# Gabrielcb/DaliID

Hardware: AMD Instinct MI355X
Metric: images/sec (train step) (higher is better)
Workload: dtype bf16; 1 GPU; configs[1]: ResNet-50 ReID bf16 256x128, PK batch 16x16=256 per GPU, center+proxy heads, Adam, EMA; global_batch=256, per_gpu_batch=256, parallelism=dp1

## Files before the change

daliid_amd/_lib.py:

```python
import ctypes
import os
import threading

import torch

_HERE = os.path.dirname(os.path.abspath(__file__))
LIB_PATH = os.environ.get("DALIID_LIB") or os.path.join(_HERE, "libdaliid_hip.so")

c_void_p, c_int, c_float, c_size_t = ctypes.c_void_p, ctypes.c_int, ctypes.c_float, ctypes.c_size_t


class DaliError(RuntimeError):
    pass


_SIGNATURES = {
    "dali_version": [],
    "dali_last_error": [],
    "dali_ctx_create": [c_int, ctypes.POINTER(c_void_p)],
    "dali_ctx_destroy": [c_void_p],
    "dali_ctx_reserve": [c_void_p, c_size_t],
    "dali_comm_unique_id": [c_void_p],
    "dali_ctx_comm_init": [c_void_p, c_void_p, c_int, c_int],
    "dali_ctx_comm_destroy": [c_void_p],
# ... 47 lines not shown
    "dali_linear_wgrad": [c_void_p] * 6 + [c_int] * 3,
    "dali_vit_patchify": [c_void_p, c_void_p, c_void_p] + [c_int] * 5 + [c_void_p],
    "dali_vit_assemble_tokens": [c_void_p] * 5 + [c_int] * 3 + [c_void_p],
    "dali_vit_assemble_tokens_bwd": [c_void_p] * 3 + [c_int] * 3 + [c_void_p] * 3,
    "dali_layernorm_fwd": [c_void_p] * 5 + [c_int, c_int, c_float] + [c_void_p] * 3,
    "dali_layernorm_bwd": [c_void_p] * 8 + [c_int, c_int] + [c_void_p] * 3,
    "dali_attention_fwd": [c_void_p] * 3 + [c_int] * 4 + [c_float, c_void_p, c_void_p],
    "dali_attention_bwd": [c_void_p] * 6 + [c_int] * 4 + [c_float, c_void_p],
    "dali_center_loss_fwd": [c_void_p] * 6 + [c_float, c_int, c_int, c_void_p, c_void_p],
    "dali_center_loss_bwd": [c_void_p] * 6 + [c_float, c_int, c_int, c_void_p, c_float, c_void_p],
    "dali_proxy_loss_fwd": [c_void_p] * 6 + [c_float, c_int, c_int] + [c_void_p] * 5,
    "dali_proxy_loss_bwd": [c_void_p] * 5 + [c_int, c_int, c_void_p, c_float, c_int, c_void_p],
    "dali_proxy_kmax": [],
    "dali_adam_step": [c_void_p] * 6 + [ctypes.c_int64, c_float, c_float, c_float, c_float, c_float, c_int, c_float, c_void_p],
    "dali_ema_update": [c_void_p, c_void_p, c_void_p, c_void_p, ctypes.c_int64, c_float],
    "dali_triplet_loss_fwd": [c_void_p, c_void_p, c_void_p, c_void_p, c_void_p, c_float, c_int, c_void_p, c_void_p, c_void_p, c_void_p,
                              c_void_p],
    "dali_triplet_loss_bwd": [c_void_p, c_void_p, c_void_p, c_void_p, c_int, c_void_p, c_float, c_void_p],
    "dali_pairdist_blend": [c_void_p, c_void_p, c_void_p, c_void_p, c_int, c_int, c_int, c_int, c_int, c_void_p, c_void_p, c_void_p,
                            c_void_p, c_void_p],
    "dali_class_targets": [c_void_p, c_void_p, c_void_p, c_int, c_int, c_void_p, c_void_p, c_int, c_void_p, c_int, c_void_p, c_void_p,
                           c_void_p, c_void_p],
    "dali_resize_bicubic_u8": [c_void_p] * 7 + [c_int, c_int, c_void_p, c_void_p, c_int, c_void_p, c_void_p, c_int, c_int, c_int, c_void_p],
    "dali_augment_batch": [c_void_p, c_void_p, c_void_p, c_void_p, c_int, c_int, c_int, ctypes.POINTER(c_float), ctypes.POINTER(c_float), c_void_p],
    "dali_gemm_profile_begin": [c_void_p, c_int],
    "dali_gemm_profile_end": [c_void_p, c_void_p, c_void_p, c_void_p],
    "dali_resnet_create": [c_void_p, c_void_p, ctypes.POINTER(c_void_p)],
    "dali_resnet_destroy": [c_void_p],
    "dali_resnet_set_feature": [c_void_p, c_int],
    "dali_resnet_sizes": [c_void_p] + [c_void_p] * 6,
# ... 114 lines not shown
```

daliid_amd/csrc/eval.hip:

```cpp
#include "gemm_tile.h"
#include "topk_key.h"
#include <cstdlib>
#include <type_traits>

namespace dali {

__global__ __launch_bounds__(256) void rows_prep_kernel(const float* __restrict__ x, int n, int d, int Kp,
                                                         int normalize, float eps, uint16_t* __restrict__ img,
                                                         int layout, float* __restrict__ sq,
                                                         float* __restrict__ yout, float* __restrict__ norms) {
    const int lane = threadIdx.x & 63;
    const int row = blockIdx.x * 4 + (threadIdx.x >> 6);
    if (row >= n) return;
    const float* xr = x + (size_t)row * d;
    float ss = 0.f;
    const bool vec = (d & 3) == 0 && ((reinterpret_cast<uintptr_t>(x) & 15) == 0);
    if (vec && Kp == d && d <= 2048 && !yout && img) {
        float4 v4[8];
#pragma unroll
        for (int k = 0; k < 8; ++k) {
            const int c = lane * 4 + k * 256;
            v4[k] = c < d ? *reinterpret_cast<const float4*>(xr + c) : make_float4(0.f, 0.f, 0.f, 0.f);
        }
#pragma unroll
// ... 888 lines not shown

namespace dali {
int pairdist_dma_max_rows(int d, bool split) { return (int)((0x7ff00000ll - 1) / ((long long)pair_pitch(d, split) * 2)); }
int launch_pairdist_matrix(int num_cus, hipStream_t st, const uint16_t* g_img, const float* gsq, const uint16_t* q_img, const float* qsq, int nq, int ng,
                           int d, int metric, bool split, float* out, const int* gate) {
    if (!gate) return launch_pairdist(num_cus, st, g_img, gsq, q_img, qsq, nq, ng, d, metric, split, out);
    return launch_pairdist_dma(num_cus, st, g_img, gsq, q_img, qsq, nq, ng, d, metric, split, out, PairGate{gate});
}
int launch_pairdist_select(int num_cus, hipStream_t st, const uint16_t* g_img, const float* gsq, const uint16_t* q_img, const float* qsq, int nq, int ng,
                           int d, int metric, bool split, const PairTopk& sel) {
    return launch_pairdist_dma(num_cus, st, g_img, gsq, q_img, qsq, nq, ng, d, metric, split, (float*)nullptr, sel);
}
}

namespace dali {
template <int D>
__global__ __launch_bounds__(256) void dot_small_kernel(const float* __restrict__ Q, int ldq, const float* __restrict__ G, int ldg, int nq, int ng, int K,
                                                        float* __restrict__ out, int ldo) {
    __shared__ float red[3][16][64];
    const int lane = threadIdx.x & 63, wave = threadIdx.x >> 6, i = lane & 31, h = lane >> 5;
    const int m0 = blockIdx.y * 32, n0 = blockIdx.x * 32;
    const float* ap = Q + (size_t)min(m0 + i, nq - 1) * ldq + 8 * h;
    const float* bp = G + (size_t)min(n0 + i, ng - 1) * ldg + 8 * h;
    f32x16_t acc;
#pragma unroll
    for (int r = 0; r < 16; ++r) acc[r] = 0.f;
    const int nfull = K >> 4;
    const int ns = (nfull + 3) >> 2;
    struct Raw { float4 a0, a1, b0, b1; };
    auto load = [&](int j, Raw& st) {
        const int sc = min(wave + 4 * j, nfull - 1);
        st.a0 = *reinterpret_cast<const float4*>(ap + 16 * sc); st.a1 = *reinterpret_cast<const float4*>(ap + 16 * sc + 4);
        st.b0 = *reinterpret_cast<const float4*>(bp + 16 * sc); st.b1 = *reinterpret_cast<const float4*>(bp + 16 * sc + 4);
    };
    auto fma = [&](const Raw& st, int j) {
        const float z = wave + 4 * j < nfull ? 1.f : 0.f;
        const float a[8] = {st.a0.x * z, st.a0.y * z, st.a0.z * z, st.a0.w * z, st.a1.x * z, st.a1.y * z, st.a1.z * z, st.a1.w * z};
        const float b[8] = {st.b0.x, st.b0.y, st.b0.z, st.b0.w, st.b1.x, st.b1.y, st.b1.z, st.b1.w};
#pragma unroll
        for (int t = 0; t < 8; ++t) acc = __builtin_amdgcn_mfma_f32_32x32x2f32(a[t], b[t], acc, 0, 0, 0);
    };
    if (nfull > 0) {
        Raw ring[D];
#pragma unroll
        for (int d = 0; d < D; ++d) load(d, ring[d]);
        for (int j0 = 0; j0 < ns; j0 += D) {
#pragma unroll
            for (int d = 0; d < D; ++d) {
                fma(ring[d], j0 + d);
                load(j0 + d + D, ring[d]);
            }
        }
    }
    if ((K & 15) && wave == 0) {
#pragma unroll
        for (int t = 0; t < 8; ++t) {
            const int k = 16 * nfull + 8 * h + t;
            const float a = k < K ? ap[16 * nfull + t] : 0.f, b = k < K ? bp[16 * nfull + t] : 0.f;
            acc = __builtin_amdgcn_mfma_f32_32x32x2f32(a, b, acc, 0, 0, 0);
        }
    }
    if (wave > 0) {
#pragma unroll
        for (int r = 0; r < 16; ++r) red[wave - 1][r][lane] = acc[r];
    }
    __syncthreads();
    if (wave == 0) {
        const int n = n0 + i;
#pragma unroll
        for (int r = 0; r < 16; ++r) {
            const int m = m0 + (r & 3) + 8 * (r >> 2) + 4 * h;
            const float v = ((acc[r] + red[0][r][lane]) + red[1][r][lane]) + red[2][r][lane];
            if (m < nq && n < ng) out[(size_t)m * ldo + n] = v;
        }
    }
}
static bool dot_small_applies(int num_cus, int nq, int ng, int d, int metric, int precision, int normalize) {
    if (metric != DALI_METRIC_DOT || normalize || precision != DALI_PREC_BF16X3 || d < 16) return false;
    const long long big_tiles = (long long)((nq + 127) / 128) * ((ng + 255) / 256);
    return big_tiles * 4 <= num_cus && DALI_ENV_INT("DALI_PAIRDIST_SMALL", 1) != 0;
}
static int launch_dot_small(hipStream_t st, const float* Q, const float* G, int nq, int ng, int d, float* out) {
    const dim3 grid((ng + 31) / 32, (nq + 31) / 32);
    const int turns = ((d >> 4) + 3) >> 2;
    if (turns >= 8) hipLaunchKernelGGL(dot_small_kernel<8>, grid, dim3(256), 0, st, Q, d, G, d, nq, ng, d, out, ng);
    else if (turns >= 4) hipLaunchKernelGGL(dot_small_kernel<4>, grid, dim3(256), 0, st, Q, d, G, d, nq, ng, d, out, ng);
    else hipLaunchKernelGGL(dot_small_kernel<2>, grid, dim3(256), 0, st, Q, d, G, d, nq, ng, d, out, ng);
    DALI_LAUNCH_CHECK();
    return DALI_OK;
}
}

static int prepare_both(dali_ctx* ctx, void* stream, const float* Q, const float* G, int nq, int ng, int d, int precision, int normalize,
                        uint16_t*& g_img, uint16_t*& q_img, float*& sq) {
    const size_t g_bytes = align_up(dali_pairdist_operand_bytes(ng, d, precision), 256);
    const size_t q_bytes = align_up(dali_pairdist_operand_bytes(nq, d, precision), 256);
    char* ws = static_cast<char*>(workspace(ctx, g_bytes + q_bytes + align_up(((size_t)nq + ng) * sizeof(float), 256)));
    if (!ws) return DALI_ERR_NOMEM;
    g_img = reinterpret_cast<uint16_t*>(ws);
    q_img = reinterpret_cast<uint16_t*>(ws + g_bytes);
    sq = reinterpret_cast<float*>(ws + g_bytes + q_bytes);
    int rc = dali_pairdist_prepare(ctx, stream, G, ng, d, normalize, precision, g_img, sq);
    if (rc != DALI_OK) return rc;
    return dali_pairdist_prepare(ctx, stream, Q, nq, d, normalize, precision, q_img, sq + ng);
}

extern "C" int dali_pairdist(dali_ctx* ctx, void* stream, const float* Q, const float* G, int nq, int ng, int d,
                             int metric, int precision, int normalize, float* out) {
    DALI_REQUIRE(ctx && Q && G && out, "dali_pairdist: null argument");
    DALI_REQUIRE(nq >= 0 && ng >= 0 && d > 0, "dali_pairdist: bad shape nq=%d ng=%d d=%d", nq, ng, d);
    DALI_REQUIRE(metric == DALI_METRIC_COSINE || metric == DALI_METRIC_L2SQ || metric == DALI_METRIC_DOT, "dali_pairdist: bad metric %d", metric);
    DALI_REQUIRE(precision == DALI_PREC_BF16X3 || precision == DALI_PREC_BF16, "dali_pairdist: bad precision %d", precision);
    DALI_REQUIRE((reinterpret_cast<uintptr_t>(out) & 15) == 0, "dali_pairdist: out must be 16-byte aligned");
    if (nq == 0 || ng == 0) return DALI_OK;
    if (dot_small_applies(ctx->num_cus, nq, ng, d, metric, precision, normalize)) return launch_dot_small((hipStream_t)stream, Q, G, nq, ng, d, out);
    uint16_t *g_img, *q_img;
    float* sq;
    const int rc = prepare_both(ctx, stream, Q, G, nq, ng, d, precision, normalize, g_img, q_img, sq);
    if (rc != DALI_OK) return rc;
    return launch_pairdist(ctx->num_cus, (hipStream_t)stream, g_img, sq, q_img, sq + ng, nq, ng, d, metric, precision == DALI_PREC_BF16X3, out);
}

extern "C" int dali_pairdist_blend(dali_ctx* ctx, void* stream, const float* Q, const float* G, int nq, int ng, int d,
                                   int precision, int normalize, const float* q_mag_prev, const float* g_mag_prev,
                                   const float* q_mag, const float* g_mag, float* inout) {
    DALI_REQUIRE(ctx && Q && G && inout, "dali_pairdist_blend: null argument");
    DALI_REQUIRE(nq >= 0 && ng >= 0 && d > 0, "dali_pairdist_blend: bad shape nq=%d ng=%d d=%d", nq, ng, d);
    DALI_REQUIRE(precision == DALI_PREC_BF16X3 || precision == DALI_PREC_BF16, "dali_pairdist_blend: bad precision %d", precision);
    DALI_REQUIRE((q_mag_prev == nullptr) == (g_mag_prev == nullptr) && (q_mag == nullptr) == (g_mag == nullptr) &&
                 (q_mag_prev == nullptr) == (q_mag == nullptr),
// ... 120 lines not shown
```

daliid_amd/csrc/losses.hip:

```cpp
#include "common.h"

namespace dali {

__global__ __launch_bounds__(256) void center_rows_kernel(const float* __restrict__ S, const int32_t* __restrict__ y,
                                                           const int32_t* __restrict__ cl, const float* __restrict__ w, float inv_tau,
                                                           int nb, int NC, float* __restrict__ rowstat) {
    const int lane = threadIdx.x & 63;
    const int i = blockIdx.x * 4 + (threadIdx.x >> 6);
    if (i >= nb) return;
    const float* s = S + (size_t)i * NC;
    float m = -__builtin_inff();
    int am = 0;
#pragma unroll 4
    for (int j = lane; j < NC; j += 64) { const float v = s[j] * inv_tau; if (v > m) { m = v; am = j; } }
#pragma unroll
    for (int o = 32; o > 0; o >>= 1) {
        const float mo = __shfl_xor(m, o, 64);
        const int ao = __shfl_xor(am, o, 64);
        if (mo > m || (mo == m && ao < am)) { m = mo; am = ao; }
    }
    float se = 0.f, pos = 0.f;
    int cnt = 0;
    const int yi = y[i];
#pragma unroll 4
// ... 240 lines not shown

__global__ __launch_bounds__(256) void triplet_bwd_kernel(const int32_t* __restrict__ sel_idx, const float* __restrict__ sel_coef, int nb,
                                                           const float* __restrict__ denom, float gscale, float* __restrict__ dS_sym) {
    const size_t t = (size_t)blockIdx.x * 256 + threadIdx.x;
    if (t >= (size_t)nb * nb) return;
    const int i = (int)(t / nb), j = (int)(t % nb);
    const float z = gscale / denom[0];
    float v = 0.f;
    if (sel_idx[2 * i + 1] == j) v += sel_coef[i];
    if (sel_idx[2 * i] == j) v -= sel_coef[i];
    if (sel_idx[2 * j + 1] == i) v += sel_coef[j];
    if (sel_idx[2 * j] == i) v -= sel_coef[j];
    dS_sym[t] = v * z;
}

}

using namespace dali;

extern "C" int dali_center_loss_fwd(dali_ctx* ctx, void* stream, const float* S, const int32_t* labels, const int32_t* center_labels,
                                    const float* w, float tau, int nb, int NC, float* rowstat, float* sums) {
    DALI_REQUIRE(ctx && S && labels && center_labels && w && rowstat && sums, "dali_center_loss_fwd: null argument");
    DALI_REQUIRE(nb > 0 && NC > 0 && tau > 0.f, "dali_center_loss_fwd: bad sizes nb=%d NC=%d tau=%g", nb, NC, tau);
    hipStream_t st = (hipStream_t)stream;
    hipLaunchKernelGGL(center_rows_kernel, dim3((nb + 3) / 4), dim3(256), 0, st, S, labels, center_labels, w, 1.0f / tau, nb, NC, rowstat);
    DALI_LAUNCH_CHECK();
    hipLaunchKernelGGL(rowstat_reduce_kernel, dim3(1), dim3(256), 0, st, rowstat, nb, 4, sums);
    DALI_LAUNCH_CHECK();
    return DALI_OK;
}
// ... 44 lines not shown
    hipLaunchKernelGGL(rowstat_reduce_kernel, dim3(1), dim3(256), 0, st, rowstat, nb, 2, sums);
    DALI_LAUNCH_CHECK();
    return DALI_OK;
}

extern "C" int dali_triplet_loss_bwd(dali_ctx* ctx, void* stream, const int32_t* sel_idx, const float* sel_coef, int nb, const float* denom,
                                     float gscale, float* dS_sym) {
    DALI_REQUIRE(ctx && sel_idx && sel_coef && denom && dS_sym, "dali_triplet_loss_bwd: null argument");
    DALI_REQUIRE(nb > 0 && nb <= 32768, "dali_triplet_loss_bwd: bad batch size %d", nb);
    const size_t total = (size_t)nb * nb;
    hipLaunchKernelGGL(triplet_bwd_kernel, dim3((unsigned)((total + 255) / 256)), dim3(256), 0, (hipStream_t)stream, sel_idx, sel_coef, nb, denom,
                       gscale, dS_sym);
    DALI_LAUNCH_CHECK();
    return DALI_OK;
}
```

daliid_amd/csrc/nnops.hip:

```cpp
#include "kernels.h"
#include "reduce_finish.h"

namespace dali {

__device__ __forceinline__ void unpack8(const uint4& v, float (&f)[8]) {
    f[0] = bf16_bits_to_f32(v.x & 0xffffu); f[1] = bf16_bits_to_f32(v.x >> 16);
    f[2] = bf16_bits_to_f32(v.y & 0xffffu); f[3] = bf16_bits_to_f32(v.y >> 16);
    f[4] = bf16_bits_to_f32(v.z & 0xffffu); f[5] = bf16_bits_to_f32(v.z >> 16);
    f[6] = bf16_bits_to_f32(v.w & 0xffffu); f[7] = bf16_bits_to_f32(v.w >> 16);
}
__device__ __forceinline__ uint4 pack8(const float (&f)[8]) {
    return make_uint4(pack_bf16x2(f[0], f[1]), pack_bf16x2(f[2], f[3]), pack_bf16x2(f[4], f[5]), pack_bf16x2(f[6], f[7]));
}
__device__ __forceinline__ void load8f(const float* __restrict__ p, float (&f)[8]) {
    const float4 a = *reinterpret_cast<const float4*>(p), b = *reinterpret_cast<const float4*>(p + 4);
    f[0] = a.x; f[1] = a.y; f[2] = a.z; f[3] = a.w; f[4] = b.x; f[5] = b.y; f[6] = b.z; f[7] = b.w;
}

struct FinBnFwd {
    double count;
    const float *gamma, *beta;
    float *running_mean, *running_var;
    float momentum, eps;
    float *scale, *shift, *mean_out, *invstd_out;
// ... 555 lines not shown
            sum[t] += __shfl_xor(sum[t], o, 64);
            const float ob = __shfl_xor(best[t], o, 64);
            const int oi = __shfl_xor(bi[t], o, 64);
            if (ob > best[t] || (ob == best[t] && oi < bi[t])) { best[t] = ob; bi[t] = oi; }
        }
    if (live && sub == 0) {
#pragma unroll
        for (int t = 0; t < 8; ++t) {
            f[(size_t)n * C + cc + t] = (mode == DALI_FEATURE_GMP ? 0.f : sum[t] / (float)HW) + (mode == DALI_FEATURE_GAP ? 0.f : best[t]);
            arg[(size_t)n * C + cc + t] = (int16_t)bi[t];
        }
    }
}
__global__ __launch_bounds__(256) void head_pool_bwd_kernel(const float* __restrict__ df, const int16_t* __restrict__ arg, int N, int HW,
                                                             int C, int mode, uint16_t* __restrict__ dx, const uint8_t* __restrict__ ybits) {
    const int cpr = C >> 3;
    const unsigned total = (unsigned)N * HW * cpr;
    const bool hw_pow2 = (HW & (HW - 1)) == 0;
    const float inv_hw = 1.f / (float)HW;
    for (unsigned i = blockIdx.x * 256u + threadIdx.x; i < total; i += gridDim.x * 256u) {
        const unsigned pix = i / (unsigned)cpr;
        const int cc = (int)(i - pix * cpr) * 8;
        const int n = (int)(pix / (unsigned)HW), p = (int)(pix - (unsigned)n * HW);
        float g[8], o[8];
        load8f(df + (size_t)n * C + cc, g);
        const uint4 av = *reinterpret_cast<const uint4*>(arg + (size_t)n * C + cc);
        const int a[8] = {(int)(int16_t)(av.x & 0xffff), (int)(int16_t)(av.x >> 16), (int)(int16_t)(av.y & 0xffff), (int)(int16_t)(av.y >> 16),
                          (int)(int16_t)(av.z & 0xffff), (int)(int16_t)(av.z >> 16), (int)(int16_t)(av.w & 0xffff), (int)(int16_t)(av.w >> 16)};
#pragma unroll
        for (int t = 0; t < 8; ++t) {
            const float avg = hw_pow2 ? g[t] * inv_hw : g[t] / (float)HW;
            o[t] = (mode == DALI_FEATURE_GMP ? 0.f : avg) + ((mode != DALI_FEATURE_GAP && a[t] == p) ? g[t] : 0.f);
        }
        if (ybits) {
            const unsigned m = ybits[((size_t)pix * C + cc) >> 3];
#pragma unroll
            for (int t = 0; t < 8; ++t) o[t] = ((m >> t) & 1u) ? o[t] : 0.f;
        }
        *reinterpret_cast<uint4*>(dx + (size_t)pix * C + cc) = pack8(o);
    }
}

__device__ __forceinline__ double bn1d_slice_sum(double v, double (*red)[32]) {
    const int cx = threadIdx.x & 31, ry = threadIdx.x >> 5;
    __syncthreads();
    red[ry][cx] = v;
    __syncthreads();
    double s = 0.0;
#pragma unroll
    for (int k = 0; k < 8; ++k) s += red[k][cx];
    return s;
}
__global__ __launch_bounds__(256) void bn1d_fwd_kernel(const float* __restrict__ x, int N, int C, const float* __restrict__ gamma,
                                                        const float* __restrict__ beta, float* __restrict__ rm, float* __restrict__ rv,
// ... 280 lines not shown
        hipLaunchKernelGGL(maxpool_bn_bwd_apply_quad_kernel, dim3(grid_for((size_t)N * Ho * Wo * (C / 8))), dim3(256), 0, st, dp, arg, raw, coef, N, H, W, C,
                           Ho, Wo, draw);
    else
        hipLaunchKernelGGL(maxpool_bn_bwd_apply_kernel, dim3(grid_for((size_t)P * (C / 8))), dim3(256), 0, st, dp, arg, raw, mean, invstd, coef, N, H,
                           W, C, Ho, Wo, draw);
    DALI_LAUNCH_CHECK();
    return DALI_OK;
}
int launch_head_pool_fwd(hipStream_t st, const uint16_t* x, int N, int HW, int C, int mode, float* f, int16_t* arg) {
    hipLaunchKernelGGL(head_pool_fwd_kernel, dim3((N * (C / 8) * 8 + 255) / 256), dim3(256), 0, st, x, N, HW, C, mode, f, arg);
    DALI_LAUNCH_CHECK();
    return DALI_OK;
}
int launch_head_pool_bwd(hipStream_t st, const float* df, const int16_t* arg, int N, int HW, int C, int mode, uint16_t* dx, const uint8_t* ybits) {
    if ((long long)N * HW * (C / 8) >= (1ll << 32)) { set_error("head_pool_bwd: more than 2^32 16-byte chunks"); return DALI_ERR_LIMIT; }
    hipLaunchKernelGGL(head_pool_bwd_kernel, dim3(grid_for((size_t)N * HW * (C / 8))), dim3(256), 0, st, df, arg, N, HW, C, mode, dx, ybits);
    DALI_LAUNCH_CHECK();
    return DALI_OK;
}
int launch_bn1d_fwd(hipStream_t st, const float* x, int N, int C, const float* gamma, const float* beta, float* rm, float* rv, int training,
                    float momentum, float eps, float* y, float* mean, float* invstd) {
    hipLaunchKernelGGL(bn1d_fwd_kernel, dim3((C + 31) / 32), dim3(256), 0, st, x, N, C, gamma, beta, rm, rv, training, momentum, eps, y, mean, invstd);
    DALI_LAUNCH_CHECK();
    return DALI_OK;
}
int launch_bn1d_bwd(hipStream_t st, const float* x, const float* dy, int N, int C, const float* gamma, const float* mean, const float* invstd,
                    float* dx, float* dgamma, float* dbeta) {
    hipLaunchKernelGGL(bn1d_bwd_kernel, dim3((C + 31) / 32), dim3(256), 0, st, x, dy, N, C, gamma, mean, invstd, dx, dgamma, dbeta);
    DALI_LAUNCH_CHECK();
    return DALI_OK;
}
// ... 101 lines not shown
                                 reinterpret_cast<double*>(ws + align_up(pf * 4, 256) + align_up((size_t)C * 12, 256)));
}

extern "C" int dali_head_pool_fwd(dali_ctx* ctx, void* stream, const uint16_t* x, int n, int hw, int C, int mode, float* f, int16_t* arg) {
    DALI_REQUIRE(ctx && x && f && arg, "dali_head_pool_fwd: null argument");
    DALI_REQUIRE(mode >= DALI_FEATURE_BOTH && mode <= DALI_FEATURE_GMP, "dali_head_pool_fwd: bad feature mode %d", mode);
    DALI_REQUIRE(C % 8 == 0 && hw > 0 && hw < 32768, "dali_head_pool_fwd: bad shape");
    return launch_head_pool_fwd((hipStream_t)stream, x, n, hw, C, mode, f, arg);
}
extern "C" int dali_head_pool_bwd(dali_ctx* ctx, void* stream, const float* df, const int16_t* arg, int n, int hw, int C, int mode, uint16_t* dx) {
    DALI_REQUIRE(ctx && df && arg && dx, "dali_head_pool_bwd: null argument");
    DALI_REQUIRE(mode >= DALI_FEATURE_BOTH && mode <= DALI_FEATURE_GMP, "dali_head_pool_bwd: bad feature mode %d", mode);
    DALI_REQUIRE(C % 8 == 0 && hw > 0, "dali_head_pool_bwd: bad shape");
    return launch_head_pool_bwd((hipStream_t)stream, df, arg, n, hw, C, mode, dx);
}
extern "C" int dali_bn1d_fwd(dali_ctx* ctx, void* stream, const float* x, int n, int C, const float* gamma, const float* beta,
                             float* running_mean, float* running_var, int training, float momentum, float eps, float* y, float* mean,
                             float* invstd) {
    DALI_REQUIRE(ctx && x && gamma && beta && y, "dali_bn1d_fwd: null argument");
    DALI_REQUIRE(training || (running_mean && running_var), "dali_bn1d_fwd: eval mode needs running statistics");
    return launch_bn1d_fwd((hipStream_t)stream, x, n, C, gamma, beta, running_mean, running_var, training, momentum, eps, y, mean, invstd);
}
extern "C" int dali_bn1d_bwd(dali_ctx* ctx, void* stream, const float* x, const float* dy, int n, int C, const float* gamma,
                             const float* mean, const float* invstd, float* dx, float* dgamma, float* dbeta) {
    DALI_REQUIRE(ctx && x && dy && gamma && mean && invstd && dx && dgamma && dbeta, "dali_bn1d_bwd: null argument");
    return launch_bn1d_bwd((hipStream_t)stream, x, dy, n, C, gamma, mean, invstd, dx, dgamma, dbeta);
}
```

daliid_amd/csrc/optim.hip:

```cpp
#include "common.h"

namespace dali {

__global__ __launch_bounds__(256) void adam_kernel(float* __restrict__ p, const float* __restrict__ g, float* __restrict__ m,
                                                    float* __restrict__ v, size_t n, float lr, float beta1, float beta2, float eps,
                                                    float weight_decay, float bc1, float bc2_sqrt, float grad_scale,
                                                    float* __restrict__ wsum_partial) {
    float local = 0.f;
    const float step_size = lr / bc1;
    for (size_t i = ((size_t)blockIdx.x * 256 + threadIdx.x) * 4; i < n; i += (size_t)gridDim.x * 1024) {
        float4 pv = *reinterpret_cast<const float4*>(p + i);
        float4 gv = *reinterpret_cast<const float4*>(g + i);
        float4 mv = *reinterpret_cast<const float4*>(m + i);
        float4 vv = *reinterpret_cast<const float4*>(v + i);
        float* pp = reinterpret_cast<float*>(&pv); float* gp = reinterpret_cast<float*>(&gv);
        float* mp = reinterpret_cast<float*>(&mv); float* vp = reinterpret_cast<float*>(&vv);
#pragma unroll
        for (int t = 0; t < 4; ++t) {
            const float gg = gp[t] * grad_scale + weight_decay * pp[t];
            mp[t] = beta1 * mp[t] + (1.f - beta1) * gg;
            vp[t] = beta2 * vp[t] + (1.f - beta2) * gg * gg;
            const float denom = sqrtf(vp[t]) / bc2_sqrt + eps;
            pp[t] = pp[t] - step_size * (mp[t] / denom);
            local += pp[t] * pp[t];
// ... 19 lines not shown
    __syncthreads();
    for (int o = 128; o > 0; o >>= 1) { if (threadIdx.x < o) red[threadIdx.x] += red[threadIdx.x + o]; __syncthreads(); }
    if (threadIdx.x == 0) out[0] = (float)red[0];
}

__global__ __launch_bounds__(256) void ema_kernel(float* __restrict__ m, const float* __restrict__ theta, size_t n, float beta) {
    const float omb = 1.f - beta;
    for (size_t i = ((size_t)blockIdx.x * 256 + threadIdx.x) * 4; i < n; i += (size_t)gridDim.x * 1024) {
        float4 a = *reinterpret_cast<const float4*>(m + i);
        const float4 b = *reinterpret_cast<const float4*>(theta + i);
        a.x = beta * a.x + omb * b.x; a.y = beta * a.y + omb * b.y; a.z = beta * a.z + omb * b.z; a.w = beta * a.w + omb * b.w;
        *reinterpret_cast<float4*>(m + i) = a;
    }
}

}

using namespace dali;

extern "C" int dali_adam_step(dali_ctx* ctx, void* stream, float* params, const float* grads, float* exp_avg, float* exp_avg_sq,
                              int64_t n, float lr, float beta1, float beta2, float eps, float weight_decay, int step, float grad_scale,
                              float* weights_sqsum) {
    DALI_REQUIRE(ctx && params && grads && exp_avg && exp_avg_sq, "dali_adam_step: null argument");
    DALI_REQUIRE(n > 0 && n % 4 == 0 && step >= 1, "dali_adam_step: n must be a positive multiple of 4 and step >= 1 (n=%lld step=%d)", (long long)n, step);
    DALI_REQUIRE(((reinterpret_cast<uintptr_t>(params) | reinterpret_cast<uintptr_t>(grads) | reinterpret_cast<uintptr_t>(exp_avg) |
                   reinterpret_cast<uintptr_t>(exp_avg_sq)) & 15) == 0, "dali_adam_step: buffers must be 16-byte aligned");
    hipStream_t st = (hipStream_t)stream;
    size_t blocks = ((size_t)n / 4 + 255) / 256;
    if (blocks > 2048) blocks = 2048;
    float* partial = nullptr;
// ... 11 lines not shown
        DALI_LAUNCH_CHECK();
    }
    return DALI_OK;
}

extern "C" int dali_ema_update(dali_ctx* ctx, void* stream, float* momentum, const float* online, int64_t n, float beta) {
    DALI_REQUIRE(ctx && momentum && online, "dali_ema_update: null argument");
    DALI_REQUIRE(n > 0 && n % 4 == 0, "dali_ema_update: n must be a positive multiple of 4");
    DALI_REQUIRE(((reinterpret_cast<uintptr_t>(momentum) | reinterpret_cast<uintptr_t>(online)) & 15) == 0, "dali_ema_update: buffers must be 16-byte aligned");
    size_t blocks = ((size_t)n / 4 + 255) / 256;
    if (blocks > 2048) blocks = 2048;
    hipLaunchKernelGGL(ema_kernel, dim3((unsigned)blocks), dim3(256), 0, (hipStream_t)stream, momentum, online, (size_t)n, beta);
    DALI_LAUNCH_CHECK();
    return DALI_OK;
}
```

daliid_amd/optim.py:

```python
import torch

from . import _lib


def _param_table(net):
    base, out = net.flat_params.data_ptr(), []
    for name, p in net.named_parameters():
        out.append((name, p, (p.data_ptr() - base) // 4, p.numel()))
    return out


def active_ranges(net, params=None):
    table = _param_table(net)
    no_grad = set(getattr(net, "_no_grad_params", ()))
    if params is None:
        chosen = {id(p) for _, p, _, _ in table if p.requires_grad}
    else:
        by_ptr = {p.data_ptr(): p for _, p, _, _ in table}
        chosen = set()
        for q in params:
            m = by_ptr.get(q.data_ptr())
            if m is None:
                raise _lib.DaliError("FusedAdam: an optimizer parameter is not a view of this net's flat parameter buffer")
            chosen.add(id(m))
# ... 79 lines not shown
        if frozen is None:
            self.weights_sqsum = self._sq[0:1]
        else:
            self.weights_sqsum = self._sq.sum().reshape(1) + frozen
        net.mark_weights_changed()
        if frozen is not None:
            self._frozen_key = net.flat_params._version


def ema_update(momentum_net, online_net, beta):
    L = _lib.lib()
    dev = online_net.flat_params.device
    for m, o in ((momentum_net.flat_params, online_net.flat_params), (momentum_net.flat_buffers, online_net.flat_buffers)):
        _lib.check(L.dali_ema_update(_lib.ctx(dev), _lib.stream_ptr(), _lib.ptr(m), _lib.ptr(o), m.numel(), float(beta)), "dali_ema_update")
    momentum_net.mark_weights_changed()
    momentum_net.flat_nbt.copy_((beta * momentum_net.flat_nbt.double() + (1 - beta) * online_net.flat_nbt.double()).to(torch.long))
```

daliid_amd/train_encodersKIT.py:

```python
import numpy as np
import torch

from . import _lib, ops_eval, optim, parallel
from .getFeatures import extractFeatures, get_image_loader
from .losses import LossHeads, _codes, _sample_weights

np.random.seed(12)
torch.manual_seed(12)

_train_loader = None


def set_train_loader(fn):
    global _train_loader
    _train_loader = fn


def get_train_loader():
    if _train_loader is not None:
        return _train_loader
    from .transforms import gpu_train_loader
    return gpu_train_loader


# ... 156 lines not shown
        emb = net._run_forward(batch_imgs, training=True)
        fn = ops_eval.l2norm_rows(emb, 1e-9)
        stats, dfn = heads(fn, labels_codes, w)
        d_emb = ops_eval.l2norm_rows_bwd(emb, dfn, 1e-9)
        n_stages = net.n_bwd_stages
        if self.process_group is not None and self._dp is None:
            self._dp = parallel.GradReducer(net.flat_grads, [net._bwd_plan.stage_range(s) for s in range(n_stages)], self.process_group)
        for stage in range(n_stages):
            net._backward_stage(d_emb, stage)
            if self._dp is not None:
                self._dp.reduce_stage(stage)
        if self._dp is not None:
            self._dp.finish()
        self._adam.step()
        optim.ema_update(self._mom, net, self.beta)
        total, lc, lp = LossHeads.losses_from_stats(stats, self.lambda_proxy)
        acc[0] += lc; acc[1] += lp; acc[2] += total
        acc[3:4] += self._adam.weights_sqsum
        acc[4] += 1
        return stats

    def train(self, selected_images, selected_labels, number_of_iterations, current_epoch):
        dev = torch.device("cuda", self.gpu_indexes[0])
        event_dataset = samplePKBatches(self.dataset, selected_images, selected_labels, self.img_height, self.img_width,
                                        self.turbulance_dir_path, self.kind_of_transform, K=self.K)
        num_classes = np.unique(selected_labels).shape[0]
        bs = min(self.P, num_classes)
        world = rank = 0
        if self.process_group is not None:
            import torch.distributed as dist
            world, rank = dist.get_world_size(self.process_group), dist.get_rank(self.process_group)
            if bs % world != 0 or bs < 3:
                raise _lib.DaliError("data parallel: P=%d identities per batch must be >= 3 and divide over %d ranks" % (bs, world))
            event_dataset.labels_set = parallel.broadcast_from_rank0(event_dataset.labels_set, self.process_group)
# ... 42 lines not shown
```

include/daliid.h:

```cpp
#ifndef DALIID_H
#define DALIID_H

#include <stddef.h>
#include <stdint.h>

#ifdef __cplusplus
extern "C" {
#endif

typedef enum {
    DALI_OK = 0,
    DALI_ERR_INVALID = -1,
    DALI_ERR_HIP = -2,
    DALI_ERR_NOMEM = -3,
    DALI_ERR_LIMIT = -4,
    DALI_ERR_UNSUPPORTED = -5
} dali_status;

typedef struct dali_ctx dali_ctx;

int dali_version(void);
const char* dali_last_error(void);
int dali_ctx_create(int device, dali_ctx** out);
int dali_ctx_destroy(dali_ctx* ctx);
// ... 144 lines not shown
                        const float* w, float tau, int nb, int NP, float* rowstat, float* sums, int32_t* sel_idx,
                        float* sel_coef, int32_t* status);
int dali_proxy_loss_bwd(dali_ctx* ctx, void* stream, const int32_t* sel_idx, const float* sel_coef, const float* proxies, int nb,
                        int D, const float* denom, float gscale, int accumulate, float* dfn);
int dali_proxy_kmax(void);

int dali_comm_unique_id(void* id128);
int dali_ctx_comm_init(dali_ctx* ctx, const void* id128, int rank, int world);
int dali_ctx_comm_destroy(dali_ctx* ctx);
int dali_allreduce_bucket(dali_ctx* ctx, void* stream, float* buf, int64_t count);

int dali_adam_step(dali_ctx* ctx, void* stream, float* params, const float* grads, float* exp_avg, float* exp_avg_sq,
                   int64_t n, float lr, float beta1, float beta2, float eps, float weight_decay, int step, float grad_scale,
                   float* weights_sqsum);
int dali_ema_update(dali_ctx* ctx, void* stream, float* momentum, const float* online, int64_t n, float beta);

int dali_triplet_loss_fwd(dali_ctx* ctx, void* stream, const float* S, const int32_t* labels, const float* w, float tau, int nb,
                          float* rowstat, float* sums, int32_t* sel_idx, float* sel_coef, int32_t* status);
int dali_triplet_loss_bwd(dali_ctx* ctx, void* stream, const int32_t* sel_idx, const float* sel_coef, int nb, const float* denom,
                          float gscale, float* dS_sym);

int dali_class_targets(dali_ctx* ctx, void* stream, const float* fvs, int n, int d, const int32_t* order,
                       const int32_t* bounds, int n_classes, const int32_t* first_pick, int num_proxies,
                       float* centers, float* proxies, int32_t* proxy_rows, float* max_dist);

int dali_resize_bicubic_u8(dali_ctx* ctx, void* stream, const uint8_t* src, const int64_t* src_off, const int32_t* in_h,
                           const int32_t* in_w, const int32_t* table_of, int n, int max_in_h, const int32_t* bounds_h,
                           const int32_t* coefs_h, int ksize_h, const int32_t* bounds_v, const int32_t* coefs_v, int ksize_v,
                           int out_h, int out_w, uint8_t* out);
int dali_augment_batch(dali_ctx* ctx, void* stream, const uint8_t* images, const int32_t* params, int n, int h, int w,
// ... 55 lines not shown
```

include/daliid_debug.h:

```cpp
#ifndef DALIID_DEBUG_H
#define DALIID_DEBUG_H

#ifdef __cplusplus
extern "C" {
#endif

int dali_debug_reload_env(void);

int dali_debug_set_conv_stamps(void* dev_ptr);

int dali_debug_wgrad_splits(int Cm, int Ntot, int P, int taps, int halo_w);

int dali_debug_splitk_reduce(void* stream, const float* partial, float* out, long long elems, int splits, int accumulate);

struct dali_resnet;
int dali_debug_resnet_backward_block(struct dali_resnet* net, void* stream, const float* d_emb, int block);

#ifdef __cplusplus
}
#endif
#endif
```

Measured before the change: 17300 images/s.

## Move EMA counters and loss accumulation to GPU kernels; retile small dot and pool bwd

Replaces the torch-side EMA update of the batch-norm counters and the per-step loss/weight accumulator with two small HIP kernels. This cuts several small torch launches and dtype-conversion ops per step. Separately, the small pairwise-dot kernel gains 2x1, 1x2 and 2x2 register tiles chosen by grid size. The head pooling backward is unrolled four ways and gets a quarter of the grid, raising memory-level parallelism at the cost of register pressure.

Measured after the change: 17380 images/s (median of 6 runs). Within noise of the previous version (+0.4%).

```diff
diff --git a/daliid_amd/_lib.py b/daliid_amd/_lib.py
--- a/daliid_amd/_lib.py
+++ b/daliid_amd/_lib.py
@@ -85,6 +85,8 @@
     "dali_proxy_kmax": [],
     "dali_adam_step": [c_void_p] * 6 + [ctypes.c_int64, c_float, c_float, c_float, c_float, c_float, c_int, c_float, c_void_p],
     "dali_ema_update": [c_void_p, c_void_p, c_void_p, c_void_p, ctypes.c_int64, c_float],
+    "dali_ema_update_counters": [c_void_p, c_void_p, c_void_p, c_void_p, ctypes.c_int64, ctypes.c_double],
+    "dali_train_acc_update": [c_void_p, c_void_p, c_void_p, c_float, c_void_p, c_void_p],
     "dali_triplet_loss_fwd": [c_void_p, c_void_p, c_void_p, c_void_p, c_void_p, c_float, c_int, c_void_p, c_void_p, c_void_p, c_void_p,
                               c_void_p],
     "dali_triplet_loss_bwd": [c_void_p, c_void_p, c_void_p, c_void_p, c_int, c_void_p, c_float, c_void_p],
diff --git a/daliid_amd/csrc/eval.hip b/daliid_amd/csrc/eval.hip
--- a/daliid_amd/csrc/eval.hip
+++ b/daliid_amd/csrc/eval.hip
@@ -926,41 +926,72 @@
 }
 
 namespace dali {
-template <int D>
+template <int D, int BM, int BN>
 __global__ __launch_bounds__(256) void dot_small_kernel(const float* __restrict__ Q, int ldq, const float* __restrict__ G, int ldg, int nq, int ng, int K,
                                                         float* __restrict__ out, int ldo) {
-    __shared__ float red[3][16][64];
+    __shared__ float red[3][BM * BN][16][64];
     const int lane = threadIdx.x & 63, wave = threadIdx.x >> 6, i = lane & 31, h = lane >> 5;
-    const int m0 = blockIdx.y * 32, n0 = blockIdx.x * 32;
-    const float* ap = Q + (size_t)min(m0 + i, nq - 1) * ldq + 8 * h;
-    const float* bp = G + (size_t)min(n0 + i, ng - 1) * ldg + 8 * h;
-    f32x16_t acc;
-#pragma unroll
-    for (int r = 0; r < 16; ++r) acc[r] = 0.f;
+    const int m0 = blockIdx.y * (32 * BM), n0 = blockIdx.x * (32 * BN);
+    const float* ap[BM];
+    const float* bp[BN];
+#pragma unroll
+    for (int bi = 0; bi < BM; ++bi) ap[bi] = Q + (size_t)min(m0 + 32 * bi + i, nq - 1) * ldq + 8 * h;
+#pragma unroll
+    for (int bj = 0; bj < BN; ++bj) bp[bj] = G + (size_t)min(n0 + 32 * bj + i, ng - 1) * ldg + 8 * h;
+    f32x16_t acc[BM][BN];
+#pragma unroll
+    for (int bi = 0; bi < BM; ++bi)
+#pragma unroll
+        for (int bj = 0; bj < BN; ++bj)
+#pragma unroll
+            for (int r = 0; r < 16; ++r) acc[bi][bj][r] = 0.f;
     const int nfull = K >> 4;
     const int ns = (nfull + 3) >> 2;
-    struct Raw { float4 a0, a1, b0, b1; };
+    struct Raw { float4 a[BM][2], b[BN][2]; };
     auto load = [&](int j, Raw& st) {
         const int sc = min(wave + 4 * j, nfull - 1);
-        st.a0 = *reinterpret_cast<const float4*>(ap + 16 * sc); st.a1 = *reinterpret_cast<const float4*>(ap + 16 * sc + 4);
-        st.b0 = *reinterpret_cast<const float4*>(bp + 16 * sc); st.b1 = *reinterpret_cast<const float4*>(bp + 16 * sc + 4);
+#pragma unroll
+        for (int bi = 0; bi < BM; ++bi) {
+            st.a[bi][0] = *reinterpret_cast<const float4*>(ap[bi] + 16 * sc); st.a[bi][1] = *reinterpret_cast<const float4*>(ap[bi] + 16 * sc + 4);
+        }
+#pragma unroll
+        for (int bj = 0; bj < BN; ++bj) {
+            st.b[bj][0] = *reinterpret_cast<const float4*>(bp[bj] + 16 * sc); st.b[bj][1] = *reinterpret_cast<const float4*>(bp[bj] + 16 * sc + 4);
+        }
     };
     auto fma = [&](const Raw& st, int j) {
         const float z = wave + 4 * j < nfull ? 1.f : 0.f;
-        const float a[8] = {st.a0.x * z, st.a0.y * z, st.a0.z * z, st.a0.w * z, st.a1.x * z, st.a1.y * z, st.a1.z * z, st.a1.w * z};
-        const float b[8] = {st.b0.x, st.b0.y, st.b0.z, st.b0.w, st.b1.x, st.b1.y, st.b1.z, st.b1.w};
-#pragma unroll
-        for (int t = 0; t < 8; ++t) acc = __builtin_amdgcn_mfma_f32_32x32x2f32(a[t], b[t], acc, 0, 0, 0);
+        float a[BM][8], b[BN][8];
+#pragma unroll
+        for (int bi = 0; bi < BM; ++bi) {
+            const float4 a0 = st.a[bi][0], a1 = st.a[bi][1];
+            a[bi][0] = a0.x * z; a[bi][1] = a0.y * z; a[bi][2] = a0.z * z; a[bi][3] = a0.w * z;
+            a[bi][4] = a1.x * z; a[bi][5] = a1.y * z; a[bi][6] = a1.z * z; a[bi][7] = a1.w * z;
+        }
+#pragma unroll
+        for (int bj = 0; bj < BN; ++bj) {
+            const float4 b0 = st.b[bj][0], b1 = st.b[bj][1];
+            b[bj][0] = b0.x; b[bj][1] = b0.y; b[bj][2] = b0.z; b[bj][3] = b0.w; b[bj][4] = b1.x; b[bj][5] = b1.y; b[bj][6] = b1.z; b[bj][7] = b1.w;
+        }
+#pragma unroll
+        for (int t = 0; t < 8; ++t)
+#pragma unroll
+            for (int bi = 0; bi < BM; ++bi)
+#pragma unroll
+                for (int bj = 0; bj < BN; ++bj) acc[bi][bj] = __builtin_amdgcn_mfma_f32_32x32x2f32(a[bi][t], b[bj][t], acc[bi][bj], 0, 0, 0);
     };
     if (nfull > 0) {
         Raw ring[D];
 #pragma unroll
         for (int d = 0; d < D; ++d) load(d, ring[d]);
+        __builtin_amdgcn_sched_barrier(0);
         for (int j0 = 0; j0 < ns; j0 += D) {
 #pragma unroll
             for (int d = 0; d < D; ++d) {
                 fma(ring[d], j0 + d);
+                __builtin_amdgcn_sched_barrier(0);
                 load(j0 + d + D, ring[d]);
+                __builtin_amdgcn_sched_barrier(0);
             }
         }
     }
@@ -968,23 +999,39 @@
 #pragma unroll
         for (int t = 0; t < 8; ++t) {
             const int k = 16 * nfull + 8 * h + t;
-            const float a = k < K ? ap[16 * nfull + t] : 0.f, b = k < K ? bp[16 * nfull + t] : 0.f;
-            acc = __builtin_amdgcn_mfma_f32_32x32x2f32(a, b, acc, 0, 0, 0);
+            float a[BM], b[BN];
+#pragma unroll
+            for (int bi = 0; bi < BM; ++bi) a[bi] = k < K ? ap[bi][16 * nfull + t] : 0.f;
+#pragma unroll
+            for (int bj = 0; bj < BN; ++bj) b[bj] = k < K ? bp[bj][16 * nfull + t] : 0.f;
+#pragma unroll
+            for (int bi = 0; bi < BM; ++bi)
+#pragma unroll
+                for (int bj = 0; bj < BN; ++bj) acc[bi][bj] = __builtin_amdgcn_mfma_f32_32x32x2f32(a[bi], b[bj], acc[bi][bj], 0, 0, 0);
         }
     }
     if (wave > 0) {
 #pragma unroll
-        for (int r = 0; r < 16; ++r) red[wave - 1][r][lane] = acc[r];
+        for (int bi = 0; bi < BM; ++bi)
+#pragma unroll
+            for (int bj = 0; bj < BN; ++bj)
+#pragma unroll
+                for (int r = 0; r < 16; ++r) red[wave - 1][bi * BN + bj][r][lane] = acc[bi][bj][r];
     }
     __syncthreads();
     if (wave == 0) {
-        const int n = n0 + i;
-#pragma unroll
-        for (int r = 0; r < 16; ++r) {
-            const int m = m0 + (r & 3) + 8 * (r >> 2) + 4 * h;
-            const float v = ((acc[r] + red[0][r][lane]) + red[1][r][lane]) + red[2][r][lane];
-            if (m < nq && n < ng) out[(size_t)m * ldo + n] = v;
-        }
+#pragma unroll
+        for (int bi = 0; bi < BM; ++bi)
+#pragma unroll
+            for (int bj = 0; bj < BN; ++bj) {
+                const int n = n0 + 32 * bj + i, blk = bi * BN + bj;
+#pragma unroll
+                for (int r = 0; r < 16; ++r) {
+                    const int m = m0 + 32 * bi + (r & 3) + 8 * (r >> 2) + 4 * h;
+                    const float v = ((acc[bi][bj][r] + red[0][blk][r][lane]) + red[1][blk][r][lane]) + red[2][blk][r][lane];
+                    if (m < nq && n < ng) out[(size_t)m * ldo + n] = v;
+                }
+            }
     }
 }
 static bool dot_small_applies(int num_cus, int nq, int ng, int d, int metric, int precision, int normalize) {
@@ -992,15 +1039,47 @@
     const long long big_tiles = (long long)((nq + 127) / 128) * ((ng + 255) / 256);
     return big_tiles * 4 <= num_cus && DALI_ENV_INT("DALI_PAIRDIST_SMALL", 1) != 0;
 }
-static int launch_dot_small(hipStream_t st, const float* Q, const float* G, int nq, int ng, int d, float* out) {
-    const dim3 grid((ng + 31) / 32, (nq + 31) / 32);
+struct DotTile { int bm, bn; };
+static DotTile dot_small_tile(int nq, int ng, int K, int num_cus) {
+    (void)K;
+    const long long full = 2ll * num_cus;
+    if (nq >= 64 && ng >= 64 && (long long)((nq + 63) / 64) * ((ng + 63) / 64) >= full) return {2, 2};
+    if (nq >= 64 && (long long)((nq + 63) / 64) * ((ng + 31) / 32) >= full) return {2, 1};
+    if (ng >= 64 && (long long)((nq + 31) / 32) * ((ng + 63) / 64) >= full) return {1, 2};
+    return {1, 1};
+}
+static bool dot_small_instantiated(int bm, int bn) { return (bm == 1 || bm == 2) && (bn == 1 || bn == 2); }
+template <int BM, int BN>
+static void launch_dot_small_tile(hipStream_t st, const float* Q, const float* G, int nq, int ng, int d, float* out) {
+    const dim3 grid((ng + 32 * BN - 1) / (32 * BN), (nq + 32 * BM - 1) / (32 * BM));
     const int turns = ((d >> 4) + 3) >> 2;
-    if (turns >= 8) hipLaunchKernelGGL(dot_small_kernel<8>, grid, dim3(256), 0, st, Q, d, G, d, nq, ng, d, out, ng);
-    else if (turns >= 4) hipLaunchKernelGGL(dot_small_kernel<4>, grid, dim3(256), 0, st, Q, d, G, d, nq, ng, d, out, ng);
-    else hipLaunchKernelGGL(dot_small_kernel<2>, grid, dim3(256), 0, st, Q, d, G, d, nq, ng, d, out, ng);
+    if constexpr (BM * BN == 1) {
+        if (turns >= 8) { hipLaunchKernelGGL((dot_small_kernel<8, 1, 1>), grid, dim3(256), 0, st, Q, d, G, d, nq, ng, d, out, ng); return; }
+    }
+    if (turns >= 4) hipLaunchKernelGGL((dot_small_kernel<4, BM, BN>), grid, dim3(256), 0, st, Q, d, G, d, nq, ng, d, out, ng);
+    else hipLaunchKernelGGL((dot_small_kernel<2, BM, BN>), grid, dim3(256), 0, st, Q, d, G, d, nq, ng, d, out, ng);
+}
+static int launch_dot_small(hipStream_t st, const float* Q, const float* G, int nq, int ng, int d, DotTile t, float* out) {
+    if (t.bm == 2 && t.bn == 2) launch_dot_small_tile<2, 2>(st, Q, G, nq, ng, d, out);
+    else if (t.bm == 2) launch_dot_small_tile<2, 1>(st, Q, G, nq, ng, d, out);
+    else if (t.bn == 2) launch_dot_small_tile<1, 2>(st, Q, G, nq, ng, d, out);
+    else launch_dot_small_tile<1, 1>(st, Q, G, nq, ng, d, out);
     DALI_LAUNCH_CHECK();
     return DALI_OK;
 }
+}
+
+extern "C" int dali_debug_dot_small(dali_ctx* ctx, void* stream, const float* Q, const float* G, int nq, int ng, int d, int bm, int bn, float* out) {
+    DALI_REQUIRE(ctx && Q && G && out, "dali_debug_dot_small: null argument");
+    DALI_REQUIRE(nq > 0 && ng > 0 && d > 0, "dali_debug_dot_small: bad shape nq=%d ng=%d d=%d", nq, ng, d);
+    DALI_REQUIRE(dali::dot_small_instantiated(bm, bn), "dali_debug_dot_small: no %d x %d tile (blocks of 32: 1 or 2 each way)", bm, bn);
+    return dali::launch_dot_small((hipStream_t)stream, Q, G, nq, ng, d, dali::DotTile{bm, bn}, out);
+}
+extern "C" int dali_debug_dot_small_tile(int nq, int ng, int d, int num_cus, int* bm, int* bn) {
+    DALI_REQUIRE(bm && bn && nq > 0 && ng > 0 && d > 0 && num_cus > 0, "dali_debug_dot_small_tile: bad argument");
+    const dali::DotTile t = dali::dot_small_tile(nq, ng, d, num_cus);
+    *bm = t.bm; *bn = t.bn;
+    return DALI_OK;
 }
 
 static int prepare_both(dali_ctx* ctx, void* stream, const float* Q, const float* G, int nq, int ng, int d, int precision, int normalize,
@@ -1025,7 +1104,7 @@
     DALI_REQUIRE(precision == DALI_PREC_BF16X3 || precision == DALI_PREC_BF16, "dali_pairdist: bad precision %d", precision);
     DALI_REQUIRE((reinterpret_cast<uintptr_t>(out) & 15) == 0, "dali_pairdist: out must be 16-byte aligned");
     if (nq == 0 || ng == 0) return DALI_OK;
-    if (dot_small_applies(ctx->num_cus, nq, ng, d, metric, precision, normalize)) return launch_dot_small((hipStream_t)stream, Q, G, nq, ng, d, out);
+    if (dot_small_applies(ctx->num_cus, nq, ng, d, metric, precision, normalize)) return launch_dot_small((hipStream_t)stream, Q, G, nq, ng, d, dot_small_tile(nq, ng, d, ctx->num_cus), out);
     uint16_t *g_img, *q_img;
     float* sq;
     const int rc = prepare_both(ctx, stream, Q, G, nq, ng, d, precision, normalize, g_img, q_img, sq);
diff --git a/daliid_amd/csrc/losses.hip b/daliid_amd/csrc/losses.hip
--- a/daliid_amd/csrc/losses.hip
+++ b/daliid_amd/csrc/losses.hip
@@ -278,6 +278,17 @@
     dS_sym[t] = v * z;
 }
 
+__global__ void train_acc_update_kernel(const float* __restrict__ stats, float lam, const float* __restrict__ wsq, float* __restrict__ acc) {
+    const float s0 = stats[0], s1 = stats[1], s2 = stats[2], s3 = stats[3], w = wsq[0];
+    const float a0 = acc[0], a1 = acc[1], a2 = acc[2], a3 = acc[3], a4 = acc[4];
+    const float c = __fdiv_rn(s0, s1), p = __fdiv_rn(s2, s3);
+    const float total = __fadd_rn(c, __fmul_rn(lam, p));
+    acc[0] = __fadd_rn(a0, c);
+    acc[1] = __fadd_rn(a1, p);
+    acc[2] = __fadd_rn(a2, total);
+    acc[3] = __fadd_rn(a3, w);
+    acc[4] = __fadd_rn(a4, 1.f);
+}
 }
 
 using namespace dali;
@@ -352,3 +363,10 @@
     DALI_LAUNCH_CHECK();
     return DALI_OK;
 }
+
+extern "C" int dali_train_acc_update(dali_ctx* ctx, void* stream, const float* stats, float lambda, const float* weights_sqsum, float* acc) {
+    DALI_REQUIRE(ctx && stats && weights_sqsum && acc, "dali_train_acc_update: null argument");
+    hipLaunchKernelGGL(train_acc_update_kernel, dim3(1), dim3(1), 0, (hipStream_t)stream, stats, lambda, weights_sqsum, acc);
+    DALI_LAUNCH_CHECK();
+    return DALI_OK;
+}
diff --git a/daliid_amd/csrc/nnops.hip b/daliid_amd/csrc/nnops.hip
--- a/daliid_amd/csrc/nnops.hip
+++ b/daliid_amd/csrc/nnops.hip
@@ -593,30 +593,59 @@
 }
 __global__ __launch_bounds__(256) void head_pool_bwd_kernel(const float* __restrict__ df, const int16_t* __restrict__ arg, int N, int HW,
                                                              int C, int mode, uint16_t* __restrict__ dx, const uint8_t* __restrict__ ybits) {
+    constexpr int U = 4;
     const int cpr = C >> 3;
     const unsigned total = (unsigned)N * HW * cpr;
     const bool hw_pow2 = (HW & (HW - 1)) == 0;
     const float inv_hw = 1.f / (float)HW;
-    for (unsigned i = blockIdx.x * 256u + threadIdx.x; i < total; i += gridDim.x * 256u) {
-        const unsigned pix = i / (unsigned)cpr;
-        const int cc = (int)(i - pix * cpr) * 8;
-        const int n = (int)(pix / (unsigned)HW), p = (int)(pix - (unsigned)n * HW);
-        float g[8], o[8];
-        load8f(df + (size_t)n * C + cc, g);
-        const uint4 av = *reinterpret_cast<const uint4*>(arg + (size_t)n * C + cc);
-        const int a[8] = {(int)(int16_t)(av.x & 0xffff), (int)(int16_t)(av.x >> 16), (int)(int16_t)(av.y & 0xffff), (int)(int16_t)(av.y >> 16),
-                          (int)(int16_t)(av.z & 0xffff), (int)(int16_t)(av.z >> 16), (int)(int16_t)(av.w & 0xffff), (int)(int16_t)(av.w >> 16)};
-#pragma unroll
-        for (int t = 0; t < 8; ++t) {
-            const float avg = hw_pow2 ? g[t] * inv_hw : g[t] / (float)HW;
-            o[t] = (mode == DALI_FEATURE_GMP ? 0.f : avg) + ((mode != DALI_FEATURE_GAP && a[t] == p) ? g[t] : 0.f);
+    const unsigned long long stride = (unsigned long long)gridDim.x * 256u;
+    for (unsigned long long i0 = blockIdx.x * 256u + threadIdx.x; i0 < total; i0 += U * stride) {
+        unsigned idx[U];
+        int p[U];
+        bool live[U];
+        float4 g0[U], g1[U];
+        uint4 av[U];
+        unsigned m[U];
+#pragma unroll
+        for (int u = 0; u < U; ++u) {
+            const unsigned long long iu = i0 + u * stride;
+            live[u] = iu < total;
+            const unsigned i = live[u] ? (unsigned)iu : total - 1;
+            idx[u] = i;
+            const unsigned pix = i / (unsigned)cpr;
+            const int cc = (int)(i - pix * cpr) * 8;
+            const int n = (int)(pix / (unsigned)HW);
+            p[u] = (int)(pix - (unsigned)n * HW);
+            const float* gp = df + (size_t)n * C + cc;
+            g0[u] = *reinterpret_cast<const float4*>(gp); g1[u] = *reinterpret_cast<const float4*>(gp + 4);
+            av[u] = *reinterpret_cast<const uint4*>(arg + (size_t)n * C + cc);
         }
         if (ybits) {
-            const unsigned m = ybits[((size_t)pix * C + cc) >> 3];
-#pragma unroll
-            for (int t = 0; t < 8; ++t) o[t] = ((m >> t) & 1u) ? o[t] : 0.f;
-        }
-        *reinterpret_cast<uint4*>(dx + (size_t)pix * C + cc) = pack8(o);
+#pragma unroll
+            for (int u = 0; u < U; ++u) m[u] = ybits[idx[u]];
+        } else {
+#pragma unroll
+            for (int u = 0; u < U; ++u) m[u] = 0xffu;
+        }
+        auto finish = [&](auto pow2) {
+#pragma unroll
+            for (int u = 0; u < U; ++u) {
+                const float g[8] = {g0[u].x, g0[u].y, g0[u].z, g0[u].w, g1[u].x, g1[u].y, g1[u].z, g1[u].w};
+                const uint4 v = av[u];
+                const int a[8] = {(int)(int16_t)(v.x & 0xffff), (int)(int16_t)(v.x >> 16), (int)(int16_t)(v.y & 0xffff), (int)(int16_t)(v.y >> 16),
+                                  (int)(int16_t)(v.z & 0xffff), (int)(int16_t)(v.z >> 16), (int)(int16_t)(v.w & 0xffff), (int)(int16_t)(v.w >> 16)};
+                float o[8];
+#pragma unroll
+                for (int t = 0; t < 8; ++t) {
+                    const float avg = decltype(pow2)::value ? g[t] * inv_hw : g[t] / (float)HW;
+                    o[t] = (mode == DALI_FEATURE_GMP ? 0.f : avg) + ((mode != DALI_FEATURE_GAP && a[t] == p[u]) ? g[t] : 0.f);
+                    o[t] = ((m[u] >> t) & 1u) ? o[t] : 0.f;
+                }
+                if (live[u]) *reinterpret_cast<uint4*>(dx + (size_t)idx[u] * 8) = pack8(o);
+            }
+        };
+        if (hw_pow2) finish(std::true_type{});
+        else finish(std::false_type{});
     }
 }
 
@@ -927,7 +956,7 @@
 }
 int launch_head_pool_bwd(hipStream_t st, const float* df, const int16_t* arg, int N, int HW, int C, int mode, uint16_t* dx, const uint8_t* ybits) {
     if ((long long)N * HW * (C / 8) >= (1ll << 32)) { set_error("head_pool_bwd: more than 2^32 16-byte chunks"); return DALI_ERR_LIMIT; }
-    hipLaunchKernelGGL(head_pool_bwd_kernel, dim3(grid_for((size_t)N * HW * (C / 8))), dim3(256), 0, st, df, arg, N, HW, C, mode, dx, ybits);
+    hipLaunchKernelGGL(head_pool_bwd_kernel, dim3(grid_for(((size_t)N * HW * (C / 8) + 3) / 4)), dim3(256), 0, st, df, arg, N, HW, C, mode, dx, ybits);
     DALI_LAUNCH_CHECK();
     return DALI_OK;
 }
@@ -1059,6 +1088,13 @@
     DALI_REQUIRE(C % 8 == 0 && hw > 0, "dali_head_pool_bwd: bad shape");
     return launch_head_pool_bwd((hipStream_t)stream, df, arg, n, hw, C, mode, dx);
 }
+extern "C" int dali_debug_head_pool_bwd(void* stream, const float* df, const int16_t* arg, int n, int hw, int C, int mode, const uint8_t* ybits,
+                                        uint16_t* dx) {
+    DALI_REQUIRE(df && arg && dx, "dali_debug_head_pool_bwd: null argument");
+    DALI_REQUIRE(mode >= DALI_FEATURE_BOTH && mode <= DALI_FEATURE_GMP, "dali_debug_head_pool_bwd: bad feature mode %d", mode);
+    DALI_REQUIRE(C % 8 == 0 && hw > 0 && n > 0, "dali_debug_head_pool_bwd: bad shape");
+    return launch_head_pool_bwd((hipStream_t)stream, df, arg, n, hw, C, mode, dx, ybits);
+}
 extern "C" int dali_bn1d_fwd(dali_ctx* ctx, void* stream, const float* x, int n, int C, const float* gamma, const float* beta,
                              float* running_mean, float* running_var, int training, float momentum, float eps, float* y, float* mean,
                              float* invstd) {
diff --git a/daliid_amd/csrc/optim.hip b/daliid_amd/csrc/optim.hip
--- a/daliid_amd/csrc/optim.hip
+++ b/daliid_amd/csrc/optim.hip
@@ -57,6 +57,11 @@
     }
 }
 
+__global__ __launch_bounds__(256) void ema_counters_kernel(long long* __restrict__ m, const long long* __restrict__ o, int n, double beta, double omb) {
+    const int i = blockIdx.x * 256 + threadIdx.x;
+    if (i < n) m[i] = (long long)__dadd_rn(__dmul_rn(beta, __ll2double_rn(m[i])), __dmul_rn(omb, __ll2double_rn(o[i])));
+}
+
 }
 
 using namespace dali;
@@ -98,3 +103,13 @@
     DALI_LAUNCH_CHECK();
     return DALI_OK;
 }
+
+extern "C" int dali_ema_update_counters(dali_ctx* ctx, void* stream, int64_t* momentum, const int64_t* online, int64_t n, double beta) {
+    DALI_REQUIRE(ctx && (n == 0 || (momentum && online)), "dali_ema_update_counters: null argument");
+    DALI_REQUIRE(n >= 0 && n < (1ll << 30), "dali_ema_update_counters: bad count %lld", (long long)n);
+    if (n == 0) return DALI_OK;
+    hipLaunchKernelGGL(ema_counters_kernel, dim3((unsigned)((n + 255) / 256)), dim3(256), 0, (hipStream_t)stream, reinterpret_cast<long long*>(momentum),
+                       reinterpret_cast<const long long*>(online), (int)n, beta, 1.0 - beta);
+    DALI_LAUNCH_CHECK();
+    return DALI_OK;
+}
diff --git a/daliid_amd/optim.py b/daliid_amd/optim.py
--- a/daliid_amd/optim.py
+++ b/daliid_amd/optim.py
@@ -117,4 +117,6 @@
     for m, o in ((momentum_net.flat_params, online_net.flat_params), (momentum_net.flat_buffers, online_net.flat_buffers)):
         _lib.check(L.dali_ema_update(_lib.ctx(dev), _lib.stream_ptr(), _lib.ptr(m), _lib.ptr(o), m.numel(), float(beta)), "dali_ema_update")
     momentum_net.mark_weights_changed()
-    momentum_net.flat_nbt.copy_((beta * momentum_net.flat_nbt.double() + (1 - beta) * online_net.flat_nbt.double()).to(torch.long))
+    nbt_m, nbt_o = momentum_net.flat_nbt, online_net.flat_nbt
+    _lib.check(L.dali_ema_update_counters(_lib.ctx(dev), _lib.stream_ptr(), _lib.ptr(nbt_m, torch.long), _lib.ptr(nbt_o, torch.long), nbt_m.numel(),
+                                          float(beta)), "dali_ema_update_counters")
diff --git a/daliid_amd/train_encodersKIT.py b/daliid_amd/train_encodersKIT.py
--- a/daliid_amd/train_encodersKIT.py
+++ b/daliid_amd/train_encodersKIT.py
@@ -194,10 +194,9 @@
             self._dp.finish()
         self._adam.step()
         optim.ema_update(self._mom, net, self.beta)
-        total, lc, lp = LossHeads.losses_from_stats(stats, self.lambda_proxy)
-        acc[0] += lc; acc[1] += lp; acc[2] += total
-        acc[3:4] += self._adam.weights_sqsum
-        acc[4] += 1
+        _lib.check(_lib.lib().dali_train_acc_update(_lib.ctx(acc.device), _lib.stream_ptr(), _lib.ptr(stats, torch.float32), float(self.lambda_proxy),
+                                                    _lib.ptr(self._adam.weights_sqsum, torch.float32), _lib.ptr(acc, torch.float32)),
+                   "dali_train_acc_update")
         return stats
 
     def train(self, selected_images, selected_labels, number_of_iterations, current_epoch):
diff --git a/include/daliid.h b/include/daliid.h
--- a/include/daliid.h
+++ b/include/daliid.h
@@ -182,6 +182,8 @@
                    int64_t n, float lr, float beta1, float beta2, float eps, float weight_decay, int step, float grad_scale,
                    float* weights_sqsum);
 int dali_ema_update(dali_ctx* ctx, void* stream, float* momentum, const float* online, int64_t n, float beta);
+int dali_ema_update_counters(dali_ctx* ctx, void* stream, int64_t* momentum, const int64_t* online, int64_t n, double beta);
+int dali_train_acc_update(dali_ctx* ctx, void* stream, const float* stats, float lambda, const float* weights_sqsum, float* acc);
 
 int dali_triplet_loss_fwd(dali_ctx* ctx, void* stream, const float* S, const int32_t* labels, const float* w, float tau, int nb,
                           float* rowstat, float* sums, int32_t* sel_idx, float* sel_coef, int32_t* status);
diff --git a/include/daliid_debug.h b/include/daliid_debug.h
--- a/include/daliid_debug.h
+++ b/include/daliid_debug.h
@@ -16,6 +16,14 @@
 struct dali_resnet;
 int dali_debug_resnet_backward_block(struct dali_resnet* net, void* stream, const float* d_emb, int block);
 
+struct dali_ctx;
+int dali_debug_dot_small(struct dali_ctx* ctx, void* stream, const float* Q, const float* G, int nq, int ng, int d, int bm, int bn, float* out);
+
+int dali_debug_dot_small_tile(int nq, int ng, int d, int num_cus, int* bm, int* bn);
+
+int dali_debug_head_pool_bwd(void* stream, const float* df, const short* arg, int n, int hw, int C, int mode, const unsigned char* ybits,
+                             unsigned short* dx);
+
 #ifdef __cplusplus
 }
 #endif
```
